# ksahlin/NGSpeciesID

Measured on AMD Instinct MI355X. Metric: reads/sec end-to-end (cluster + spoa consensus + racon x3), 750 bp ONT, higher is better.
Workload: dtype u8 / int16 / int32 DP, 64-bit bit-vectors (f64 thresholds)

## Files before the change

### ngspeciesid_amd/csrc/k_align.hip

```cpp
#include "k_align_common.h"
#include <algorithm>
#include <type_traits>

#define NEGINF (-(1 << 29))

template <int RPL>
__global__ __launch_bounds__(256) __attribute__((amdgpu_waves_per_eu(3, 4)))
void k_sg_align(AlignJob J, uint64_t* __restrict__ tb, uint64_t tb_words_per_wave, int32_t* __restrict__ bnd, uint32_t bnd_stride, uint32_t lds_per_wave, uint32_t* __restrict__ work_ctr)
{
    extern __shared__ __attribute__((aligned(16))) unsigned char smem[];
    const int lane = threadIdx.x & 63;
    const int wib = threadIdx.x >> 6;
    const uint64_t wave = (uint64_t)blockIdx.x * (blockDim.x >> 6) + wib;
    uint8_t* tgt = smem + (size_t)wib * lds_per_wave;
    const uint32_t seq_lds = (lds_per_wave - 4096) / 2;
    uint8_t* qry = tgt + seq_lds;
    uint64_t* tbblk = (uint64_t*)(tgt + 2 * (size_t)seq_lds);
    uint64_t* mytb = tb + wave * tb_words_per_wave;
    int32_t* mybnd = bnd + wave * (uint64_t)bnd_stride * 2;
    const int STRIP = 64 * RPL;

    for (;;) {
        uint32_t pq = 0; if (lane == 0) pq = atomicAdd(work_ctr, 1u);
        const uint64_t px = (uint32_t)__builtin_amdgcn_readfirstlane((int)pq);
// ... 183 lines not shown
static int32_t plan16(ngsid_ctx* ctx, uint64_t npairs, uint32_t max_qlen, uint32_t max_tlen, StripPlan* L)
{
    return plan_strips(ctx, (const void*)k_sg_align16<RP>, 2 * RP, 127, npairs, max_qlen, max_tlen, L);
}
template <int RP>
static int32_t launch16(ngsid_ctx* ctx, const AlignJob& job, const StripPlan& L, hipStream_t st, uint32_t* ctr, uint64_t* tb, int32_t* bnd)
{
    { ProfScope ps_(ctx, st == ctx->stream ? "k_sg_align" : "k_sg_align_side", st);
      hipLaunchKernelGGL((k_sg_align16<RP>), dim3((unsigned)(L.nwaves / L.wpb)), dim3(64 * L.wpb), (size_t)L.wpb * L.lds_per_wave, st,
                         job, tb, L.words, bnd, L.bnd_stride, L.lds_per_wave, ctr); }
    HIPCHK(ctx, hipGetLastError());
    return NGSID_OK;
}

struct PairedPlan { uint64_t words_half, nwaves; uint32_t seq_lds; size_t lds; };
template <int R>
static int32_t plan16p(ngsid_ctx* ctx, uint64_t npairs, uint32_t max_tlen, PairedPlan* L)
{
    L->seq_lds = (std::max<uint32_t>(max_tlen, 64u * R) + 15u) & ~15u;
    L->lds = 4 * (size_t)L->seq_lds + 4096;
    L->words_half = ((uint64_t)max_tlen + 63) * 64;
    return plan_waves(ctx, (const void*)k_sg_align16p<R>, 1, L->lds, (npairs + 1) / 2, 2 * L->words_half * 8, &L->nwaves);
}

__global__ __launch_bounds__(256)
void k_pair_bins(AlignJob J, const uint32_t* __restrict__ list, const uint32_t* __restrict__ count, int R, uint8_t* __restrict__ bin_of, uint32_t* __restrict__ bin_cnt )
{
    const uint32_t k = blockIdx.x * blockDim.x + threadIdx.x;
    const int lane = threadIdx.x & 63;
    int bin = -1;
    if (k < *count) {
        const uint64_t p = list[k]; const uint32_t qi = J.qidx[p];
        const int n = (int)(J.qoff[qi + 1] - J.qoff[qi]);
        bin = n >= 1 ? (n - 1) % R : 0;
        bin_of[k] = (uint8_t)bin;
    }
    for (int b = 0; b < PBINS; ++b) {
// ... 12 lines not shown
void k_bin_scatter(const uint32_t* __restrict__ list, const uint32_t* __restrict__ count, const uint8_t* __restrict__ bin_of, const uint32_t* __restrict__ bin_off, uint32_t* __restrict__ cursor, uint32_t* __restrict__ sorted)
{
    const uint32_t k = blockIdx.x * blockDim.x + threadIdx.x;
    const int lane = threadIdx.x & 63;
    const int bin = k < *count ? (int)bin_of[k] : -1;
    for (int b = 0; b < PBINS; ++b) {
        const unsigned long long mk = __ballot(bin == b);
        if (!mk) continue;
        const int leader = (int)__builtin_ctzll(mk);
        uint32_t base = 0; if (lane == leader) base = atomicAdd(&cursor[b], (uint32_t)__popcll(mk));
        base = __shfl(base, leader);
        if (bin == b) sorted[bin_off[b] + base + __popcll(mk & ((1ull << lane) - 1))] = list[k];
    }
}

template <int R>
static int32_t launch16p(ngsid_ctx* ctx, const AlignJob& job, int cls, uint32_t max_tlen, hipStream_t st, uint64_t* tb)
{
    const uint64_t n = job.npairs;
    const size_t ints = 4 * PBINS + 8;
    if (ctx->aln_pint.n < 4 * ints) HIPCHK(ctx, ctx->aln_pint.alloc(4 * ints));
    if (ctx->aln_psorted.n < 4 * n) HIPCHK(ctx, ctx->aln_psorted.reserve(4 * n));
    if (ctx->aln_pbin.n < 4 * n) HIPCHK(ctx, ctx->aln_pbin.reserve(4 * n));
    uint32_t* ibase = ctx->aln_pint.p + cls * ints; uint32_t* sorted = ctx->aln_psorted.p + (size_t)cls * n; uint8_t* bin_of = ctx->aln_pbin.p + (size_t)cls * n;
    const uint32_t* list = ctx->aln_cls.p + (size_t)cls * n; const uint32_t* count = ctx->aln_ctr.p + 8 + cls;
    uint32_t* bin_cnt = ibase, *bin_off = ibase + PBINS, *item_off = bin_off + PBINS + 1, *cursor = item_off + PBINS + 1, *wctr = cursor + PBINS;
    HIPCHK(ctx, hipMemsetAsync(ibase, 0, (size_t)(4 * PBINS + 8) * sizeof(uint32_t), st));
    const unsigned nb = (unsigned)((n + 255) / 256);
    hipLaunchKernelGGL(k_pair_bins, dim3(nb), dim3(256), 0, st, job, list, count, R, bin_of, bin_cnt);
    hipLaunchKernelGGL(k_bin_offsets, dim3(1), dim3(64), 0, st, (const uint32_t*)bin_cnt, bin_off, item_off, cursor);
    hipLaunchKernelGGL(k_bin_scatter, dim3(nb), dim3(256), 0, st, list, count, (const uint8_t*)bin_of, (const uint32_t*)bin_off, cursor, sorted);
    HIPCHK(ctx, hipGetLastError());
    PairedPlan L; int32_t rc = plan16p<R>(ctx, n, max_tlen, &L); if (rc) return rc;
    HIPCHK(ctx, hipFuncSetAttribute((const void*)k_sg_align16p<R>, hipFuncAttributeMaxDynamicSharedMemorySize, (int)L.lds));
    { ProfScope ps_(ctx, st == ctx->stream ? "k_sg_align" : "k_sg_align_side", st);
      hipLaunchKernelGGL((k_sg_align16p<R>), dim3((unsigned)L.nwaves), dim3(64), L.lds, st, job, (const uint32_t*)sorted, (const uint32_t*)bin_off, (const uint32_t*)item_off, tb, L.words_half, L.seq_lds, wctr); }
    HIPCHK(ctx, hipGetLastError());
    return NGSID_OK;
}


#define NCLS 5
struct AlignClass { uint32_t bound; int rp, r, side; };
constexpr AlignClass kAlignClass[NCLS] = {{256, 2, 4, 0}, {512, 4, 8, 1}, {768, 6, 12, -1}, {896, 7, 14, 2}, {0xffffffffu, 8, 0, 3}};

template <class F>
static int32_t with_class(int c, F&& f)
{
    switch (c) {
        case 0: return f(std::integral_constant<int, 0>{});
        case 1: return f(std::integral_constant<int, 1>{});
// ... 23 lines not shown
        if (cls == c) lists[(size_t)c * J.npairs + base + __popcll(m & ((1ull << lane) - 1))] = (uint32_t)p;
    }
}

int32_t ngsid_partition_pairs(ngsid_ctx* ctx, const AlignJob& job, uint32_t long_len)
{
    const uint64_t n = job.npairs;
    if (ctx->aln_ctr.n < 16) HIPCHK(ctx, ctx->aln_ctr.alloc(16));
    if (ctx->aln_cls.n < (size_t)(NCLS + 1) * n) HIPCHK(ctx, ctx->aln_cls.reserve((size_t)(NCLS + 1) * n));
    HIPCHK(ctx, hipMemsetAsync(ctx->aln_ctr.p, 0, 16 * sizeof(uint32_t), ctx->stream));
    hipLaunchKernelGGL(k_pair_classes, dim3((unsigned)((n + 255) / 256)), dim3(256), 0, ctx->stream, job, ctx->aln_cls.p, ctx->aln_ctr.p + 8, long_len);
    HIPCHK(ctx, hipGetLastError());
    return NGSID_OK;
}

static int32_t launch_classes(ngsid_ctx* ctx, const AlignJob& job, uint32_t max_qlen, uint32_t max_tlen, uint32_t min_qlen, uint32_t long_len)
{
    const uint64_t n = job.npairs;
    { int32_t rc = ngsid_partition_pairs(ctx, job, long_len); if (rc) return rc; }
    { int32_t rc = ngsid_side_streams(ctx); if (rc) return rc; }
    const bool paired = ngsid_opt(ctx, "align_paired", 1) != 0;
    bool used[NCLS]; uint64_t tbo[NCLS + 1] = {0}, bo[NCLS + 1] = {0};
    for (int c = 0; c < NCLS; ++c) {
        used[c] = (c == 0 || max_qlen > kAlignClass[c - 1].bound) && min_qlen <= std::min(max_qlen, kAlignClass[c].bound);
        uint64_t words = 0, bwords = 0;
        if (used[c]) {
            int32_t rc = with_class(c, [&](auto C) -> int32_t {
                constexpr AlignClass K = kAlignClass[decltype(C)::value];
                if constexpr (K.r > 0) {
                    if (paired) { PairedPlan P; int32_t r = plan16p<K.r>(ctx, n, max_tlen, &P); words = P.nwaves * 2 * P.words_half; return r; }
                }
                StripPlan L; int32_t r = plan16<K.rp>(ctx, n, std::min(max_qlen, K.bound), max_tlen, &L); words = L.nwaves * L.words; bwords = L.nwaves * 2ull * L.bnd_stride; return r;
            });
            if (rc) return rc;
        }
        tbo[c + 1] = tbo[c] + words; bo[c + 1] = bo[c] + bwords;
    }
    if (ctx->tb.n < tbo[NCLS]) HIPCHK(ctx, ctx->tb.reserve(tbo[NCLS]));
    if (ctx->bnd.n < bo[NCLS]) HIPCHK(ctx, ctx->bnd.reserve(bo[NCLS]));
    HIPCHK(ctx, hipEventRecord(ctx->ev_fork, ctx->stream));
    for (int i = 0; i < 4; ++i) HIPCHK(ctx, hipStreamWaitEvent(ctx->side[i], ctx->ev_fork, 0));
    for (int on_main = 0; on_main < 2; ++on_main)
        for (int c = 0; c < NCLS; ++c) {
            if (!used[c] || (kAlignClass[c].side < 0) != (on_main == 1)) continue;
            const hipStream_t st = kAlignClass[c].side < 0 ? ctx->stream : ctx->side[kAlignClass[c].side];
            int32_t rc = with_class(c, [&](auto C) -> int32_t {
                constexpr AlignClass K = kAlignClass[decltype(C)::value];
                if constexpr (K.r > 0) {
                    if (paired) return launch16p<K.r>(ctx, job, c, max_tlen, st, ctx->tb.p + tbo[c]);
                }
                AlignJob jc = job; jc.pair_list = ctx->aln_cls.p + (size_t)c * n; jc.npairs_dev = ctx->aln_ctr.p + 8 + c;
                StripPlan L; int32_t r = plan16<K.rp>(ctx, n, std::min(max_qlen, K.bound), max_tlen, &L); if (r) return r;
                return launch16<K.rp>(ctx, jc, L, st, ctx->aln_ctr.p + 1 + c, ctx->tb.p + tbo[c], ctx->bnd.p + bo[c]);
            });
            if (rc) return rc;
        }
    for (int i = 0; i < 4; ++i) { HIPCHK(ctx, hipEventRecord(ctx->ev_join[i], ctx->side[i])); HIPCHK(ctx, hipStreamWaitEvent(ctx->stream, ctx->ev_join[i], 0)); }
    return NGSID_OK;
}

bool ngsid_align16_applicable(const AlignJob& job, uint32_t max_qlen, uint32_t max_tlen, int max_open)
{
    return max_qlen <= NGSID_ALIGN16_MAXLEN && max_tlen <= NGSID_ALIGN16_MAXLEN && job.match >= 0 && job.match <= 4 && job.mismatch <= 0 && job.mismatch >= -8 &&
           job.ext >= 0 && job.ext <= 4 && max_open >= 0 && max_open <= 16;
}

__global__ __launch_bounds__(256) void k_align_cells(AlignJob J, unsigned long long* __restrict__ stat)
{
    const uint64_t np = J.npairs_dev ? (uint64_t)*J.npairs_dev : J.npairs;
    unsigned long long c = 0;
    for (uint64_t x = (uint64_t)blockIdx.x * 256 + threadIdx.x; x < np; x += (uint64_t)gridDim.x * 256) {
        const uint64_t p = J.pair_list ? J.pair_list[x] : x; const uint32_t qi = J.qidx[p], ti = J.tidx[p];
        c += (unsigned long long)(J.qoff[qi + 1] - J.qoff[qi]) * (unsigned long long)(J.toff[ti + 1] - J.toff[ti]);
    }
#pragma unroll
    for (int d = 32; d >= 1; d >>= 1) c += __shfl_xor(c, d);
    __shared__ unsigned long long part[4];
    if ((threadIdx.x & 63) == 0) part[threadIdx.x >> 6] = c;
    __syncthreads();
    if (threadIdx.x == 0) atomicAdd(stat, part[0] + part[1] + part[2] + part[3]);
}

int32_t ngsid_launch_align(ngsid_ctx* ctx, const AlignJob& job, uint32_t max_qlen, uint32_t max_tlen, int max_open, uint32_t min_qlen)
{
    if (job.npairs == 0) return NGSID_OK;
    if (ctx->prof && ctx->stat.p && !job.bp) { hipLaunchKernelGGL(k_align_cells, dim3((unsigned)std::min<uint64_t>(1024, (job.npairs + 255) / 256)), dim3(256), 0, ctx->stream, job, ctx->stat.p + 1); HIPCHK(ctx, hipGetLastError()); }
    if (job.npairs > 0xf0000000ull) NGSID_FAIL(ctx, NGSID_ERR_ARG, "more than 2^32 pairs in one aligner call");
    if (max_tlen > NGSID_MAX_READ_LEN || max_qlen > NGSID_MAX_READ_LEN) NGSID_FAIL(ctx, NGSID_ERR_TOO_LONG, "sequence longer than %d in aligner", NGSID_MAX_READ_LEN);
    if (job.k > 64) NGSID_FAIL(ctx, NGSID_ERR_ARG, "window k > 64 unsupported");
    if (!job.ops && !ngsid_opt(ctx, "align32", 0)) {
        const uint32_t q16 = std::min<uint32_t>(max_qlen, NGSID_ALIGN16_MAXLEN), t16 = std::min<uint32_t>(max_tlen, NGSID_ALIGN16_MAXLEN);
        const bool has_long = max_qlen > q16 || max_tlen > t16;
        if (ngsid_align16_applicable(job, q16, t16, max_open)) {
            if (job.npairs >= 4096 && q16 > 256 && !job.pair_list && !ngsid_opt(ctx, "align_noclass", 0)) {
                int32_t rc = launch_classes(ctx, job, q16, t16, min_qlen, has_long ? NGSID_ALIGN16_MAXLEN : 0);
                if (rc || !has_long) return rc;
                AlignJob jl = job; jl.pair_list = ctx->aln_cls.p + (size_t)NCLS * job.npairs; jl.npairs_dev = ctx->aln_ctr.p + 8 + NCLS;
                return launch_rpl<16>(ctx, jl, max_qlen, max_tlen, true);
            }
            if (!has_long) {
                int c = 0; while (max_qlen > kAlignClass[c].bound) ++c;
                return with_class(c, [&](auto C) -> int32_t {
                    constexpr int RP = kAlignClass[decltype(C)::value].rp;
                    StripPlan L; int32_t rc = plan16<RP>(ctx, job.npairs, max_qlen, max_tlen, &L); if (rc) return rc;
                    if (ctx->aln_ctr.n < 16) HIPCHK(ctx, ctx->aln_ctr.alloc(16));
                    HIPCHK(ctx, hipMemsetAsync(ctx->aln_ctr.p, 0, sizeof(uint32_t), ctx->stream));
                    if (ctx->tb.n < L.nwaves * L.words) HIPCHK(ctx, ctx->tb.alloc(L.nwaves * L.words));
                    if (ctx->bnd.n < L.nwaves * 2ull * L.bnd_stride) HIPCHK(ctx, ctx->bnd.alloc(L.nwaves * 2ull * L.bnd_stride));
                    return launch16<RP>(ctx, job, L, ctx->stream, ctx->aln_ctr.p, ctx->tb.p, ctx->bnd.p);
                });
// ... 11 lines not shown
```

### ngspeciesid_amd/csrc/k_align16p.hip

```cpp
#include "k_align_common.h"
#include <type_traits>

static_assert(-(NEG16) + 4  + 16  + 4  * 896  < 32768, "packed sign-bit flags of k_sg_align16p would wrap");
__device__ __forceinline__ int pp_bfi(int mask_s, int a, int b) { int d; asm("v_bfi_b32 %0, %1, %2, %3" : "=v"(d) : "s"(mask_s), "v"(a), "v"(b)); return d; }
__device__ __forceinline__ int pp_perm(int a, int b, int sel_s) { int d; asm("v_perm_b32 %0, %1, %2, %3" : "=v"(d) : "v"(a), "v"(b), "s"(sel_s)); return d; }
__device__ __forceinline__ int pp_sel(int mask, int a, int b) { return (a & mask) | (b & ~mask); }

template <int R>
struct Planes {
    const uint64_t* tb;
    __device__ SgCell at(int i, int j) const { const int l = i / R; return SgCell{l >> 3, j + l, l & 7, i - l * R}; }
    __device__ const uint64_t* block(int grp, int tt) const { return tb + (uint64_t)tt * 64 + grp * 8; }
    __device__ int flags(uint64_t word, int r) const {
        const unsigned x = (unsigned)(word >> (32 * (r >> 3) + (r & 7)));
        return (int)(~(x & 1u) & 1u) | (int)(~(x >> 7) & 2u) | (int)(~(x >> 14) & 4u) | (int)(~(x >> 21) & 8u);
    }
};

template <int R>
__global__ __launch_bounds__(64) __attribute__((amdgpu_waves_per_eu(2, 4)))
void k_sg_align16p(AlignJob J, const uint32_t* __restrict__ sorted, const uint32_t* __restrict__ bin_off , const uint32_t* __restrict__ item_off ,
                   uint64_t* __restrict__ tb, uint64_t tb_words_per_wave , uint32_t seq_lds, uint32_t* __restrict__ work_ctr)
{
    extern __shared__ __attribute__((aligned(16))) unsigned char smem[];
    const int lane = threadIdx.x;
    uint8_t* tgt0 = smem; uint8_t* tgt1 = tgt0 + seq_lds; uint8_t* qry0 = tgt1 + seq_lds; uint8_t* qry1 = qry0 + seq_lds;
    uint64_t* tbblk = (uint64_t*)(smem + 4 * (size_t)seq_lds);
    uint64_t* mytb0 = tb + (uint64_t)blockIdx.x * tb_words_per_wave * 2; uint64_t* mytb1 = mytb0 + tb_words_per_wave;
    constexpr int NA = 2 * ((R + 7) / 8);
    const uint32_t nitems = item_off[PBINS];

    for (;;) {
        uint32_t pq = 0; if (lane == 0) pq = atomicAdd(work_ctr, 1u);
        const uint32_t kq = (uint32_t)__builtin_amdgcn_readfirstlane((int)pq);
        if (kq >= nitems) break;
// ... 12 lines not shown
        if (deg0) sg_degenerate(J, p0, n0, m0, lane);
        if (deg1) sg_degenerate(J, p1, n1, m1, lane);
        const int own_p = ((n0 > 0 ? n0 : 1) - 1) % R;
        if (deg0) { n0 = 0; m0 = 0; }
        if (deg1) { n1 = 0; m1 = 0; }
        if (deg0 && (deg1 || !have1)) continue;
        unsigned wild = 0;
        for (int x = lane; x < m0; x += 64) { const uint8_t v = perm_letter(t0[x]); tgt0[x] = v; wild |= v; }
        for (int x = lane; x < n0; x += 64) { const uint8_t v = perm_letter(q0[x]); qry0[x] = v; wild |= v; }
        for (int x = lane; x < m1; x += 64) { const uint8_t v = perm_letter(t1[x]); tgt1[x] = v; wild |= v; }
        for (int x = lane; x < n1; x += 64) { const uint8_t v = perm_letter(q1[x]); qry1[x] = v; wild |= v; }
        const bool nowild = __ballot((wild & 0x7Cu) != 0) == 0;
        __builtin_amdgcn_fence(__ATOMIC_RELEASE, "workgroup");
        __builtin_amdgcn_wave_barrier();

        const int OPEN2 = sgpr(PK(J.open[p0], J.open[p1])), NOPEN2 = sgpr(PK(-J.open[p0], -J.open[p1])), EXT2 = sgpr(PK(J.ext, J.ext));
        const int MATCHO2 = PK(J.match + J.open[p0], J.match + J.open[p1]), NDIFF2 = sgpr(PK(J.mismatch - J.match, J.mismatch - J.match));
        const int ONE2 = sgpr(0x00010001);
        constexpr int SGN = 0x0B0A0908;
        constexpr int SEL0 = 0x06040200, SEL1 = 0x07050301;
        const int mmax = m0 > m1 ? m0 : m1;
        const int steps = mmax + 63;
        const int own_lane0 = n0 > 0 ? (n0 - 1) / R : -1, own_lane1 = n1 > 0 ? (n1 - 1) / R : -1;
        int bestRowV0 = -(1 << 29), bestRowJ0 = 0, bestRowV1 = -(1 << 29), bestRowJ1 = 0;
        int hl2[R], e2[R], qc2[R], nwq2[R];
        const int i0 = lane * R;
#pragma unroll
        for (int r = 0; r < R; ++r) {
            const int i = i0 + r;
            const int ca = i < n0 ? qry0[i] : 0x7C, cb = i < n1 ? qry1[i] : 0x7C;
            qc2[r] = PK(ca & 3, cb & 3); nwq2[r] = PK((ca & 0x7C) ? 0 : 0xffff, (cb & 0x7C) ? 0 : 0xffff);
            hl2[r] = NOPEN2; e2[r] = PK(NEG16, NEG16);
        }

        auto forward = [&](auto OPc, auto NWc) {
            constexpr int OWN_P = decltype(OPc)::value; constexpr bool NOWILD = decltype(NWc)::value;
            int hdiag2 = NOPEN2;
            int send_h = NOPEN2, send_f = PK(NEG16, NEG16);
            int keyRow0 = (int)0x80000000u, keyRow1 = (int)0x80000000u; const int jinv0 = 0xFFFF + lane;
            auto step = [&](int tau, auto STc) {
                constexpr bool STEADY = decltype(STc)::value;
                const int j = tau - lane;
                const int hup = __builtin_amdgcn_update_dpp(NOPEN2, send_h, 0x138, 0xf, 0xf, false), fup = __builtin_amdgcn_update_dpp(PK(NEG16, NEG16), send_f, 0x138, 0xf, 0xf, false);
                const bool a0 = STEADY || (j >= 0 && j < m0), a1 = STEADY || (j >= 0 && j < m1);
                const int l0 = tgt0[STEADY ? j : (a0 ? j : 0)], l1 = tgt1[STEADY ? j : (a1 ? j : 0)];
                const int tc2 = PK(l0 & 3, l1 & 3);
                int nwt2 = 0; if constexpr (!NOWILD) nwt2 = PK((a0 && !(l0 & 0x7C)) ? 0xffff : 0, (a1 && !(l1 & 0x7C)) ? 0xffff : 0);
                const int am2 = STEADY ? -1 : PK(a0 ? 0xffff : 0, a1 ? 0xffff : 0);
                int hu2 = hup, f2 = fup, hd2 = hdiag2;
                int acc[NA], cap2 = 0;
#pragma unroll
                for (int r = 0; r < R; ++r) {
                    const int e_ext = pk_sub_i16_s(e2[r], EXT2); const int E = pk_max_i16(e_ext, hl2[r]);
                    const int f_ext = pk_sub_i16_s(f2, EXT2); const int F = pk_max_i16(f_ext, hu2);
                    const int z = pk_min_u16_s(qc2[r] ^ tc2, ONE2);
                    int sc = pk_mad_i16_sv(z, NDIFF2, MATCHO2);
                    if constexpr (!NOWILD) { const int nw = nwq2[r] & nwt2; sc = pp_sel(nw, sc, OPEN2); }
                    const int d = pk_add_i16(hd2, sc);
                    const int mx = pk_max_i16(E, F); const int h = pk_max_i16(d, mx);
                    const int g = pk_sub_i16_s(h, OPEN2);
                    const int s0 = pk_sub_i16(d, h), s1 = pk_sub_i16(E, mx), s2 = pk_sub_i16(e_ext, E), s3 = pk_sub_i16(f_ext, F);
                    const int pa = pp_perm(s1, s0, SGN), pb = pp_perm(s3, s2, SGN);
                    int& a01 = acc[2 * (r >> 3)]; int& a23 = acc[2 * (r >> 3) + 1];
                    if ((r & 7) == 0) { a01 = pa & 0x01010101; a23 = pb & 0x01010101; }
                    else { a01 = pp_bfi(0x01010101 << (r & 7), pa, a01); a23 = pp_bfi(0x01010101 << (r & 7), pb, a23); }
                    hd2 = hl2[r];
                    hl2[r] = STEADY ? g : pp_sel(am2, g, hl2[r]);
                    e2[r] = E;
                    hu2 = g; f2 = F;
                    if (r == OWN_P) cap2 = g;
                }
                unsigned long long w0 = 0, w1 = 0;
#pragma unroll
                for (int k = 0; k < NA / 2; ++k) {
                    w0 |= (unsigned long long)(unsigned)pp_perm(acc[2 * k + 1], acc[2 * k], SEL0) << (32 * k);
                    w1 |= (unsigned long long)(unsigned)pp_perm(acc[2 * k + 1], acc[2 * k], SEL1) << (32 * k);
                }
                mytb0[(uint64_t)tau * 64 + lane] = w0;
                mytb1[(uint64_t)tau * 64 + lane] = w1;
                if (STEADY) { hdiag2 = hup; send_h = hu2; send_f = f2; }
                else { hdiag2 = pp_sel(am2, hup, hdiag2); send_h = pp_sel(am2, hu2, send_h); send_f = pp_sel(am2, f2, send_f); }
                if (STEADY) {
                    const int jinv = jinv0 - tau;
                    keyRow0 = max(keyRow0, (int)(((unsigned)cap2 << 16) | (unsigned)jinv));
                    keyRow1 = max(keyRow1, (int)(((unsigned)cap2 & 0xFFFF0000u) | (unsigned)jinv));
                } else {
                    const int v0 = LO16(cap2), v1 = HI16(cap2);
                    const bool b0_ = a0 && lane == own_lane0 && v0 > bestRowV0; bestRowV0 = b0_ ? v0 : bestRowV0; bestRowJ0 = b0_ ? j : bestRowJ0;
                    const bool b1_ = a1 && lane == own_lane1 && v1 > bestRowV1; bestRowV1 = b1_ ? v1 : bestRowV1; bestRowJ1 = b1_ ? j : bestRowJ1;
                }
            };
            const int mmin = m0 < m1 ? m0 : m1;
            const int st_lo = 63 < steps ? 63 : steps, st_hi = mmin > st_lo ? (mmin < steps ? mmin : steps) : st_lo;
            int tau = 0;
            for (; tau < st_lo; ++tau) step(tau, std::false_type{});
            for (; tau + 1 < st_hi; tau += 2) { step(tau, std::true_type{}); step(tau + 1, std::true_type{}); }
            for (; tau < st_hi; ++tau) step(tau, std::true_type{});
            if (st_hi > st_lo) {
                const int v0 = keyRow0 >> 16, v1 = keyRow1 >> 16;
                if (lane == own_lane0 && v0 > bestRowV0) { bestRowV0 = v0; bestRowJ0 = 0xFFFF - (keyRow0 & 0xFFFF); }
                if (lane == own_lane1 && v1 > bestRowV1) { bestRowV1 = v1; bestRowJ1 = 0xFFFF - (keyRow1 & 0xFFFF); }
            }
            for (; tau < steps; ++tau) step(tau, std::false_type{});
        };
        switch (own_p) {
#define PCASE(k) case k: if (nowild) forward(std::integral_constant<int, (R > k ? k : 0)>{}, std::true_type{}); else forward(std::integral_constant<int, (R > k ? k : 0)>{}, std::false_type{}); break;
            PCASE(0) PCASE(1) PCASE(2) PCASE(3) PCASE(4) PCASE(5) PCASE(6) PCASE(7) PCASE(8) PCASE(9) PCASE(10) PCASE(11) PCASE(12) PCASE(13) PCASE(14)
#undef PCASE
            default: if (nowild) forward(std::integral_constant<int, (R > 15 ? 15 : 0)>{}, std::true_type{}); else forward(std::integral_constant<int, (R > 15 ? 15 : 0)>{}, std::false_type{}); break;
        }
        bestRowV0 += LO16(OPEN2); bestRowV1 += HI16(OPEN2);
        int bestColV0 = -(1 << 29), bestColI0 = 0x7fffffff, bestColV1 = -(1 << 29), bestColI1 = 0x7fffffff;
#pragma unroll
        for (int r = 0; r < R; ++r) {
            const int i = i0 + r; const int v0 = LO16(hl2[r]) + LO16(OPEN2), v1 = HI16(hl2[r]) + HI16(OPEN2);
            if (i < n0 && v0 > bestColV0) { bestColV0 = v0; bestColI0 = i; }
            if (i < n1 && v1 > bestColV1) { bestColV1 = v1; bestColI1 = i; }
        }
        __builtin_amdgcn_fence(__ATOMIC_RELEASE, "workgroup");
        __builtin_amdgcn_s_waitcnt(0);
        __builtin_amdgcn_fence(__ATOMIC_ACQUIRE, "workgroup");

        const AlignJob* Jt = sg_cold_job();
        for (int half = 0; half < 2; ++half) {
            const uint64_t p = half ? p1 : p0; const int n = half ? n1 : n0, m = half ? m1 : m0;
            if (n <= 0) continue;
            int rowV = half ? bestRowV1 : bestRowV0, rowJ = half ? bestRowJ1 : bestRowJ0;
#pragma unroll
            for (int d = 32; d >= 1; d >>= 1) { int ov = __shfl_xor(rowV, d), oj = __shfl_xor(rowJ, d); if (ov > rowV) { rowV = ov; rowJ = oj; } }
            int colV = half ? bestColV1 : bestColV0, colI = half ? bestColI1 : bestColI0;
#pragma unroll
            for (int d = 32; d >= 1; d >>= 1) { int ov = __shfl_xor(colV, d), oi = __shfl_xor(colI, d); if (ov > colV || (ov == colV && oi < colI)) { colV = ov; colI = oi; } }
            int ei = n - 1, ej = rowJ, best = rowV;
            if (colV > best) { best = colV; ei = colI; ej = m - 1; }
            ei = sgpr(ei); ej = sgpr(ej); best = sgpr(best);
            sg_walk(Jt, Planes<R>{half ? mytb1 : mytb0}, tbblk, half ? qry1 : qry0, half ? tgt1 : tgt0, p, n, m, ei, ej, best, lane);
            __builtin_amdgcn_wave_barrier();
        }
    }
}

template __global__ void k_sg_align16p<4>(AlignJob, const uint32_t*, const uint32_t*, const uint32_t*, uint64_t*, uint64_t, uint32_t, uint32_t*);
template __global__ void k_sg_align16p<8>(AlignJob, const uint32_t*, const uint32_t*, const uint32_t*, uint64_t*, uint64_t, uint32_t, uint32_t*);
template __global__ void k_sg_align16p<12>(AlignJob, const uint32_t*, const uint32_t*, const uint32_t*, uint64_t*, uint64_t, uint32_t, uint32_t*);
template __global__ void k_sg_align16p<14>(AlignJob, const uint32_t*, const uint32_t*, const uint32_t*, uint64_t*, uint64_t, uint32_t, uint32_t*);
```

### ngspeciesid_amd/csrc/k_align_common.h

```cpp
#pragma once
#include "ngsid_internal.h"

template <int RP> __global__ void k_sg_align16(AlignJob J, uint64_t* tb, uint64_t tb_words_per_wave, int32_t* bnd, uint32_t bnd_stride, uint32_t lds_per_wave, uint32_t* work_ctr);
#define PBINS 32
template <int R> __global__ void k_sg_align16p(AlignJob J, const uint32_t* sorted, const uint32_t* bin_off, const uint32_t* item_off, uint64_t* tb, uint64_t tb_words_per_wave, uint32_t seq_lds, uint32_t* work_ctr);

#define NEG16 (-20000)
#define PKOP2(name, mnem) __device__ __forceinline__ int name(int a, int b) { int d; asm(mnem " %0, %1, %2" : "=v"(d) : "v"(a), "v"(b)); return d; }
PKOP2(pk_sub_i16, "v_pk_sub_i16")
PKOP2(pk_add_i16, "v_pk_add_i16")
PKOP2(pk_max_i16, "v_pk_max_i16")
PKOP2(pk_sub_u16, "v_pk_sub_u16")
#define PKOP2S(name, mnem) __device__ __forceinline__ int name(int a, int b) { int d; asm(mnem " %0, %1, %2" : "=v"(d) : "v"(a), "s"(b)); return d; }
PKOP2S(pk_sub_i16_s, "v_pk_sub_i16")
PKOP2S(pk_min_u16_s, "v_pk_min_u16")
__device__ __forceinline__ int pk_mad_i16_sv(int a, int b_s, int c) { int d; asm("v_pk_mad_i16 %0, %1, %2, %3" : "=v"(d) : "v"(a), "s"(b_s), "v"(c)); return d; }
__device__ __forceinline__ int sgpr(int x) { return __builtin_amdgcn_readfirstlane(x); }
__device__ __forceinline__ uint8_t perm_letter(uint8_t c) {
    const int b = ngsid_bcode(c);
    if (b < 4) return (uint8_t)(b | ((c & 0x20) ? 0x80 : 0));
    if ((c & 0x7C) == 0) { const int x = c & 3; const int up = x == 0 ? 'A' : x == 1 ? 'C' : x == 2 ? 'G' : 'T'; return (uint8_t)((c & 0x80) ? (up | 0x20) : up); }
    return c;
}
__device__ __forceinline__ int PK(int lo, int hi) { return (lo & 0xffff) | (hi << 16); }
// ... 142 lines not shown
```

### ngspeciesid_amd/csrc/ngsid_api.hip

```cpp
#include "ngsid_internal.h"
#include "../../include/ngsid_merge_schedule.h"
#include "../../include/ngsid_tables.h"
#include <math.h>
#include <algorithm>

extern "C" uint32_t ngsid_abi_version(void) { return 2u; }

static char g_static_err[256] = "";
extern "C" const char* ngsid_last_error(ngsid_ctx* ctx) { return ctx ? ctx->err : g_static_err; }

namespace {
struct DevPool { std::mutex mu; std::multimap<unsigned long long, void*> free_; size_t cached = 0; int contexts = 0; size_t live = 0, peak = 0;
                 struct Upload { size_t bs; void* q; size_t bq; void* off; size_t bo; }; std::map<void*, Upload> uploads;
};
DevPool g_pool;
const size_t POOL_LIMIT = (size_t)48 << 30;
const size_t POOL_HEADROOM = (size_t)3 << 30;
struct PoolBlocks { void* p[3] = {nullptr, nullptr, nullptr}; size_t b[3] = {0, 0, 0}; bool owned = true; ~PoolBlocks() { if (owned) for (int i = 0; i < 3; ++i) if (p[i]) ngsid_pool_free(p[i], b[i]); } };
inline size_t pool_class(size_t b) { if (b < 4096) return 4096; int sh = 63 - __builtin_clzll((unsigned long long)b) - 3; size_t m = ((size_t)1 << sh) - 1; return (b + m) & ~m; }
inline unsigned long long pool_key(int dev, size_t cls) { return ((unsigned long long)dev << 56) | (unsigned long long)cls; }
}
thread_local ngsid_ctx* g_ngsid_tls_ctx = nullptr;
hipError_t ngsid_pool_alloc(void** p, size_t bytes, size_t* got)
{
// ... 536 lines not shown
extern "C" int32_t ngsid_reads_release(ngsid_ctx* ctx, ngsid_reads_t* dev)
{
    if (!ctx) return NGSID_ERR_ARG;
    ApiClock api_clock_(ctx, "reads_release");
    if (!dev || dev->mem != NGSID_MEM_DEVICE) NGSID_FAIL(ctx, NGSID_ERR_ARG, "reads_release: not a device read set");
    DevPool::Upload u;
    { std::lock_guard<std::mutex> lk(g_pool.mu); auto it = g_pool.uploads.find((void*)dev->seq); if (it == g_pool.uploads.end()) NGSID_FAIL(ctx, NGSID_ERR_ARG, "reads_release: this read set was not made by ngsid_reads_upload (or was released already)"); u = it->second; g_pool.uploads.erase(it); }
    ngsid_pool_free((void*)dev->seq, u.bs); if (u.q) ngsid_pool_free(u.q, u.bq); ngsid_pool_free(u.off, u.bo);
    dev->seq = nullptr; dev->qual = nullptr; dev->off = nullptr; dev->n = 0;
    return NGSID_OK;
}

extern "C" int32_t ngsid_ctx_option(ngsid_ctx* ctx, const char* name, int64_t value)
{
    if (!ctx || !name) return NGSID_ERR_ARG;
    static const char* known[] = {"minimizers_chunk_bases", "poa_level_budget_mb", "cluster_block", "cluster_block_cap", "cluster_trunc", "cluster_seg_order", "ed_band", "ed_win_all", "align32", "align_noclass", "poa_tiles_per_cu", "minimizers_lean", "minimizers_mode", "poa_host_levels", "align_paired", "poa_out_slots", "ed_lds_pad_kb", "ed_win6", "support_budget_mb", "demux_chunk_reads", "classify_chunk_queries"};
    for (const char* k : known) if (!strcmp(k, name)) { ctx->options[name] = (long long)value; return NGSID_OK; }
    if (!strcmp(name, "touch")) {
        if (ctx->mzc_fp.n < 2) HIPCHK(ctx, ctx->mzc_fp.alloc(2));
        HIPCHK(ctx, hipMemsetAsync(ctx->mzc_fp.p + 1, 0, sizeof(unsigned long long), ctx->stream)); HIPCHK(ctx, hipStreamSynchronize(ctx->stream));
        return NGSID_OK;
    }
    if (!strcmp(name, "release_scratch")) {
        (void)hipStreamSynchronize(ctx->stream);
        ctx->tb.release(); ctx->bnd.release(); ctx->tb_long.release(); ctx->bnd_long.release(); ctx->aln_cls.release(); ctx->aln_psorted.release(); ctx->aln_pbin.release(); ctx->ed_tb.release(); ctx->ed_h.release(); ctx->ed_fail.release(); ctx->ed_fail2.release();
        ctx->poa_h.release(); ctx->poa_d.release(); ctx->poa_g.release(); ctx->poa_cov.release();
        for (auto& L : ctx->poa_lv) { L.out.release(); L.seqs.release(); L.job_final.release(); L.out_len.release(); L.out_span.release(); L.job_bb.release(); L.out_cw.release(); L.out_n.release(); L.out_cov.release(); L.job_off.release(); L.seq_idx.release(); L.flags.release(); L.job_list.release(); L.job_unit.release(); L.job_pos.release(); }
        ctx->mzc.valid = false; ctx->mzc_cnt.release(); ctx->mzc_hlen.release(); ctx->mz_off.release(); ctx->mz_scode.release(); ctx->mz_spos.release();
        ctx->pol_mzcode.release(); ctx->pol_mzpos.release(); ctx->pol_oseq.release(); ctx->pol_oqual.release(); ctx->pol_valid.release(); ctx->pol_bp.release(); ctx->pol_lay.release(); ctx->cl_cnt.release(); ctx->cls_cnt.release();
        ngsid_pool_release_all();
        return NGSID_OK;
// ... 56 lines not shown
```

### ngspeciesid_amd/csrc/ngsid_internal.h

```cpp
#pragma once
#include <hip/hip_runtime.h>
#include <stdint.h>
#include <stdio.h>
#include <string.h>
#include <stdlib.h>
#include <string>
#include <vector>
#include <map>
#include <new>
#include <mutex>
#include <chrono>
#include <memory>
#include <time.h>
#include "../../include/ngsid.h"

hipError_t ngsid_pool_alloc(void** p, size_t bytes, size_t* got);
void ngsid_pool_free(void* p, size_t bytes);
struct ngsid_ctx;
extern thread_local ngsid_ctx* g_ngsid_tls_ctx;
void ngsid_pool_release_all();
int ngsid_pool_contexts();
size_t ngsid_pool_cached_bytes();
void ngsid_pool_stats(size_t* live, size_t* peak, bool reset_peak);

// ... 126 lines not shown
                             uint32_t* h_cnt, uint32_t* h_hlen, long long* bad_read);

struct AlignJob {
    const uint8_t* qseq; const uint64_t* qoff; const uint8_t* tseq; const uint64_t* toff;
    const uint32_t* qidx; const uint32_t* tidx; uint64_t npairs;
    int match, mismatch, ext, k; const int32_t* open; const int32_t* match_id;
    int32_t* score; int32_t* ncols; int32_t* nmatch; int32_t* region;
    int32_t* bp; int bp_windows; int window; int32_t* span;
    const uint32_t* pair_list; const uint32_t* npairs_dev;
    uint8_t* ops; const uint64_t* ops_off;
    const uint32_t* pair_list2; const uint32_t* npairs_dev2;
    int clip;
};
int32_t ngsid_launch_align(ngsid_ctx* ctx, const AlignJob& job, uint32_t max_qlen, uint32_t max_tlen, int max_open = 1 << 20, uint32_t min_qlen = 0);
bool ngsid_align16_applicable(const AlignJob& job, uint32_t max_qlen, uint32_t max_tlen, int max_open);
#define NGSID_ALIGN16_MAXLEN 4000u
int32_t ngsid_partition_pairs(ngsid_ctx* ctx, const AlignJob& job, uint32_t long_len = 0);
int32_t ngsid_side_streams(ngsid_ctx* ctx);
int32_t ngsid_launch_ed_align(ngsid_ctx* ctx, const AlignJob& job, uint32_t max_qlen, uint32_t max_tlen, int32_t* dist_out);
int32_t ngsid_launch_ed_align_rec(ngsid_ctx* ctx, const AlignJob& job, uint32_t max_qlen, uint32_t max_tlen, uint32_t* rec, uint32_t stride);
enum { NGSID_REC_EQ = 1, NGSID_REC_SUB = 2 , NGSID_REC_OTHER = 6 , NGSID_REC_DEL = 7, NGSID_REC_INS = 8 };
struct OrientBufs { DevBuf<uint32_t> d_rgroup; DevBuf<double> herr, rawerr; DevBuf<uint8_t> d_orient; };
int32_t ngsid_polish_orient(ngsid_ctx* ctx, const DevReads& RD, const std::vector<std::string>& B, const std::vector<uint32_t>& h_rgroup, int k, int w, OrientBufs& S, PinVec<uint8_t>& h_orient);

typedef unsigned int ngsid_v4u __attribute__((ext_vector_type(4)));
__device__ __forceinline__ ngsid_v4u ngsid_load16_l2(const void* p) { return __builtin_nontemporal_load((const ngsid_v4u*)p); }

__device__ __forceinline__ int ngsid_bcode(uint8_t c) {
    switch (c) { case 'A': case 'a': return 0; case 'C': case 'c': return 1; case 'G': case 'g': return 2; case 'T': case 't': return 3; default: return 4; }
}
// ... 7 lines not shown
```

Before: 1.465 million.

## Add skewed-frame variant of paired int16 aligner with byte-permute score table

Adds a SKEW template variant of the paired 16-bit semi-global aligner. Each cell is rebased by i+j times the gap-extension cost, so the E/F extension subtracts disappear. When there are no wildcards, the match/mismatch score comes from a v_perm byte lookup table instead of xor/min/mad. It also raises the waves-per-EU hint for the skew variant. The variant is enabled by default only when a new overflow bound shows the skewed int16 range cannot wrap, and it adds extra per-step offset corrections and register pressure.

```diff
diff --git a/ngspeciesid_amd/csrc/k_align.hip b/ngspeciesid_amd/csrc/k_align.hip
--- a/ngspeciesid_amd/csrc/k_align.hip
+++ b/ngspeciesid_amd/csrc/k_align.hip
@@ -221,13 +221,13 @@
 }
 
 struct PairedPlan { uint64_t words_half, nwaves; uint32_t seq_lds; size_t lds; };
-template <int R>
+template <int R, bool SKEW>
 static int32_t plan16p(ngsid_ctx* ctx, uint64_t npairs, uint32_t max_tlen, PairedPlan* L)
 {
     L->seq_lds = (std::max<uint32_t>(max_tlen, 64u * R) + 15u) & ~15u;
     L->lds = 4 * (size_t)L->seq_lds + 4096;
     L->words_half = ((uint64_t)max_tlen + 63) * 64;
-    return plan_waves(ctx, (const void*)k_sg_align16p<R>, 1, L->lds, (npairs + 1) / 2, 2 * L->words_half * 8, &L->nwaves);
+    return plan_waves(ctx, (const void*)k_sg_align16p<R, SKEW>, 1, L->lds, (npairs + 1) / 2, 2 * L->words_half * 8, &L->nwaves);
 }
 
 __global__ __launch_bounds__(256)
@@ -270,7 +270,7 @@
     }
 }
 
-template <int R>
+template <int R, bool SKEW>
 static int32_t launch16p(ngsid_ctx* ctx, const AlignJob& job, int cls, uint32_t max_tlen, hipStream_t st, uint64_t* tb)
 {
     const uint64_t n = job.npairs;
@@ -287,10 +287,10 @@
     hipLaunchKernelGGL(k_bin_offsets, dim3(1), dim3(64), 0, st, (const uint32_t*)bin_cnt, bin_off, item_off, cursor);
     hipLaunchKernelGGL(k_bin_scatter, dim3(nb), dim3(256), 0, st, list, count, (const uint8_t*)bin_of, (const uint32_t*)bin_off, cursor, sorted);
     HIPCHK(ctx, hipGetLastError());
-    PairedPlan L; int32_t rc = plan16p<R>(ctx, n, max_tlen, &L); if (rc) return rc;
-    HIPCHK(ctx, hipFuncSetAttribute((const void*)k_sg_align16p<R>, hipFuncAttributeMaxDynamicSharedMemorySize, (int)L.lds));
+    PairedPlan L; int32_t rc = plan16p<R, SKEW>(ctx, n, max_tlen, &L); if (rc) return rc;
+    HIPCHK(ctx, hipFuncSetAttribute((const void*)k_sg_align16p<R, SKEW>, hipFuncAttributeMaxDynamicSharedMemorySize, (int)L.lds));
     { ProfScope ps_(ctx, st == ctx->stream ? "k_sg_align" : "k_sg_align_side", st);
-      hipLaunchKernelGGL((k_sg_align16p<R>), dim3((unsigned)L.nwaves), dim3(64), L.lds, st, job, (const uint32_t*)sorted, (const uint32_t*)bin_off, (const uint32_t*)item_off, tb, L.words_half, L.seq_lds, wctr); }
+      hipLaunchKernelGGL((k_sg_align16p<R, SKEW>), dim3((unsigned)L.nwaves), dim3(64), L.lds, st, job, (const uint32_t*)sorted, (const uint32_t*)bin_off, (const uint32_t*)item_off, tb, L.words_half, L.seq_lds, wctr); }
     HIPCHK(ctx, hipGetLastError());
     return NGSID_OK;
 }
@@ -344,12 +344,13 @@
     return NGSID_OK;
 }
 
-static int32_t launch_classes(ngsid_ctx* ctx, const AlignJob& job, uint32_t max_qlen, uint32_t max_tlen, uint32_t min_qlen, uint32_t long_len)
+static int32_t launch_classes(ngsid_ctx* ctx, const AlignJob& job, uint32_t max_qlen, uint32_t max_tlen, int max_open, uint32_t min_qlen, uint32_t long_len)
 {
     const uint64_t n = job.npairs;
     { int32_t rc = ngsid_partition_pairs(ctx, job, long_len); if (rc) return rc; }
     { int32_t rc = ngsid_side_streams(ctx); if (rc) return rc; }
     const bool paired = ngsid_opt(ctx, "align_paired", 1) != 0;
+    const bool skew = ngsid_opt(ctx, "align_skew", 1) != 0 && ngsid_align16p_skew_exact(job, max_qlen, max_tlen, max_open);
     bool used[NCLS]; uint64_t tbo[NCLS + 1] = {0}, bo[NCLS + 1] = {0};
     for (int c = 0; c < NCLS; ++c) {
         used[c] = (c == 0 || max_qlen > kAlignClass[c - 1].bound) && min_qlen <= std::min(max_qlen, kAlignClass[c].bound);
@@ -358,7 +359,7 @@
             int32_t rc = with_class(c, [&](auto C) -> int32_t {
                 constexpr AlignClass K = kAlignClass[decltype(C)::value];
                 if constexpr (K.r > 0) {
-                    if (paired) { PairedPlan P; int32_t r = plan16p<K.r>(ctx, n, max_tlen, &P); words = P.nwaves * 2 * P.words_half; return r; }
+                    if (paired) { PairedPlan P; int32_t r = skew ? plan16p<K.r, true>(ctx, n, max_tlen, &P) : plan16p<K.r, false>(ctx, n, max_tlen, &P); words = P.nwaves * 2 * P.words_half; return r; }
                 }
                 StripPlan L; int32_t r = plan16<K.rp>(ctx, n, std::min(max_qlen, K.bound), max_tlen, &L); words = L.nwaves * L.words; bwords = L.nwaves * 2ull * L.bnd_stride; return r;
             });
@@ -377,7 +378,7 @@
             int32_t rc = with_class(c, [&](auto C) -> int32_t {
                 constexpr AlignClass K = kAlignClass[decltype(C)::value];
                 if constexpr (K.r > 0) {
-                    if (paired) return launch16p<K.r>(ctx, job, c, max_tlen, st, ctx->tb.p + tbo[c]);
+                    if (paired) return skew ? launch16p<K.r, true>(ctx, job, c, max_tlen, st, ctx->tb.p + tbo[c]) : launch16p<K.r, false>(ctx, job, c, max_tlen, st, ctx->tb.p + tbo[c]);
                 }
                 AlignJob jc = job; jc.pair_list = ctx->aln_cls.p + (size_t)c * n; jc.npairs_dev = ctx->aln_ctr.p + 8 + c;
                 StripPlan L; int32_t r = plan16<K.rp>(ctx, n, std::min(max_qlen, K.bound), max_tlen, &L); if (r) return r;
@@ -393,6 +394,14 @@
 {
     return max_qlen <= NGSID_ALIGN16_MAXLEN && max_tlen <= NGSID_ALIGN16_MAXLEN && job.match >= 0 && job.match <= 4 && job.mismatch <= 0 && job.mismatch >= -8 &&
            job.ext >= 0 && job.ext <= 4 && max_open >= 0 && max_open <= 16;
+}
+
+bool ngsid_align16p_skew_exact(const AlignJob& job, uint32_t max_qlen, uint32_t max_tlen, int max_open)
+{
+    uint32_t qmax = 0;
+    for (int c = 0; c < NCLS; ++c) if (kAlignClass[c].r > 0) qmax = std::max(qmax, kAlignClass[c].bound);
+    return ngsid_align16_applicable(job, max_qlen, max_tlen, max_open) &&
+           sg16p_flag_span(job.match, job.ext, max_open, std::min(max_qlen, qmax), max_tlen, true) < 32768;
 }
 
 __global__ __launch_bounds__(256) void k_align_cells(AlignJob J, unsigned long long* __restrict__ stat)
@@ -423,7 +432,7 @@
         const bool has_long = max_qlen > q16 || max_tlen > t16;
         if (ngsid_align16_applicable(job, q16, t16, max_open)) {
             if (job.npairs >= 4096 && q16 > 256 && !job.pair_list && !ngsid_opt(ctx, "align_noclass", 0)) {
-                int32_t rc = launch_classes(ctx, job, q16, t16, min_qlen, has_long ? NGSID_ALIGN16_MAXLEN : 0);
+                int32_t rc = launch_classes(ctx, job, q16, t16, max_open, min_qlen, has_long ? NGSID_ALIGN16_MAXLEN : 0);
                 if (rc || !has_long) return rc;
                 AlignJob jl = job; jl.pair_list = ctx->aln_cls.p + (size_t)NCLS * job.npairs; jl.npairs_dev = ctx->aln_ctr.p + 8 + NCLS;
                 return launch_rpl<16>(ctx, jl, max_qlen, max_tlen, true);
diff --git a/ngspeciesid_amd/csrc/k_align16p.hip b/ngspeciesid_amd/csrc/k_align16p.hip
--- a/ngspeciesid_amd/csrc/k_align16p.hip
+++ b/ngspeciesid_amd/csrc/k_align16p.hip
@@ -1,9 +1,12 @@
 #include "k_align_common.h"
 #include <type_traits>
 
-static_assert(-(NEG16) + 4  + 16  + 4  * 896  < 32768, "packed sign-bit flags of k_sg_align16p would wrap");
+static_assert(sg16p_flag_span(4 , 4 , 16 , 896 , NGSID_ALIGN16_MAXLEN, false) < 32768, "packed sign-bit flags of k_sg_align16p would wrap");
+static_assert(sg16p_flag_span(4, 1, 16, 896, NGSID_ALIGN16_MAXLEN, true) < 32768, "the skewed frame of k_sg_align16p must hold every paired length with ext = 1");
 __device__ __forceinline__ int pp_bfi(int mask_s, int a, int b) { int d; asm("v_bfi_b32 %0, %1, %2, %3" : "=v"(d) : "s"(mask_s), "v"(a), "v"(b)); return d; }
 __device__ __forceinline__ int pp_perm(int a, int b, int sel_s) { int d; asm("v_perm_b32 %0, %1, %2, %3" : "=v"(d) : "v"(a), "v"(b), "s"(sel_s)); return d; }
+__device__ __forceinline__ int pp_permv(int a, int b, int sel_v) { int d; asm("v_perm_b32 %0, %1, %2, %3" : "=v"(d) : "v"(a), "v"(b), "v"(sel_v)); return d; }
+__device__ __forceinline__ int pk_ashr15_i16(int a) { int d; asm("v_pk_ashrrev_i16 %0, %1, %2" : "=v"(d) : "s"(0x000F000F), "v"(a)); return d; }
 __device__ __forceinline__ int pp_sel(int mask, int a, int b) { return (a & mask) | (b & ~mask); }
 
 template <int R>
@@ -17,8 +20,8 @@
     }
 };
 
-template <int R>
-__global__ __launch_bounds__(64) __attribute__((amdgpu_waves_per_eu(2, 4)))
+template <int R, bool SKEW>
+__global__ __launch_bounds__(64) __attribute__((amdgpu_waves_per_eu(SKEW ? (R <= 8 ? 4 : 3) : 2, 4)))
 void k_sg_align16p(AlignJob J, const uint32_t* __restrict__ sorted, const uint32_t* __restrict__ bin_off , const uint32_t* __restrict__ item_off ,
                    uint64_t* __restrict__ tb, uint64_t tb_words_per_wave , uint32_t seq_lds, uint32_t* __restrict__ work_ctr)
 {
@@ -61,9 +64,15 @@
         __builtin_amdgcn_fence(__ATOMIC_RELEASE, "workgroup");
         __builtin_amdgcn_wave_barrier();
 
-        const int OPEN2 = sgpr(PK(J.open[p0], J.open[p1])), NOPEN2 = sgpr(PK(-J.open[p0], -J.open[p1])), EXT2 = sgpr(PK(J.ext, J.ext));
-        const int MATCHO2 = PK(J.match + J.open[p0], J.match + J.open[p1]), NDIFF2 = sgpr(PK(J.mismatch - J.match, J.mismatch - J.match));
+        int ext = J.ext; if constexpr (SKEW) asm volatile("" : "+s"(ext));
+        const int open0 = sgpr(J.open[p0]), open1 = sgpr(J.open[p1]), skx = SKEW ? ext : 0;
+        const int NOPEN2 = sgpr(PK(-open0, -open1)), EXT2 = sgpr(PK(ext, ext));
+        const int dk0 = open0 + skx, dk1 = open1 + skx;
+        const int DIAG2 = sgpr(PK(dk0, dk1)), GSUB2 = sgpr(PK(open0 - skx, open1 - skx));
+        const int MATCHO2 = PK(J.match + dk0, J.match + dk1), NDIFF2 = sgpr(PK(J.mismatch - J.match, J.mismatch - J.match));
         const int ONE2 = sgpr(0x00010001);
+        const bool tbl_ok = SKEW && J.mismatch + dk0 >= 0 && J.mismatch + dk1 >= 0 && J.match + dk0 <= 255 && J.match + dk1 <= 255;
+        const int XX0 = sgpr((J.mismatch + dk0) * 0x01010101), XX1 = sgpr((J.mismatch + dk1) * 0x01010101), MX0 = sgpr((J.match + dk0) ^ (J.mismatch + dk0)), MX1 = sgpr((J.match + dk1) ^ (J.mismatch + dk1));
         constexpr int SGN = 0x0B0A0908;
         constexpr int SEL0 = 0x06040200, SEL1 = 0x07050301;
         const int mmax = m0 > m1 ? m0 : m1;
@@ -71,41 +80,53 @@
         const int own_lane0 = n0 > 0 ? (n0 - 1) / R : -1, own_lane1 = n1 > 0 ? (n1 - 1) / R : -1;
         int bestRowV0 = -(1 << 29), bestRowJ0 = 0, bestRowV1 = -(1 << 29), bestRowJ1 = 0;
         int hl2[R], e2[R], qc2[R], nwq2[R];
-        const int i0 = lane * R;
+        int i0 = lane * R; if constexpr (SKEW) asm volatile("" : "+v"(i0));
 #pragma unroll
         for (int r = 0; r < R; ++r) {
             const int i = i0 + r;
             const int ca = i < n0 ? qry0[i] : 0x7C, cb = i < n1 ? qry1[i] : 0x7C;
-            qc2[r] = PK(ca & 3, cb & 3); nwq2[r] = PK((ca & 0x7C) ? 0 : 0xffff, (cb & 0x7C) ? 0 : 0xffff);
-            hl2[r] = NOPEN2; e2[r] = PK(NEG16, NEG16);
+            if constexpr (SKEW) { qc2[r] = PK((ca & 3) | ((ca & 0x7C) ? 0x8000 : 0), (cb & 3) | ((cb & 0x7C) ? 0x8000 : 0)); nwq2[r] = 0; }
+            else { qc2[r] = PK(ca & 3, cb & 3); nwq2[r] = PK((ca & 0x7C) ? 0 : 0xffff, (cb & 0x7C) ? 0 : 0xffff); }
+            hl2[r] = SKEW ? PK(i * ext - open0, i * ext - open1) : NOPEN2; e2[r] = PK(NEG16, NEG16);
         }
 
         auto forward = [&](auto OPc, auto NWc) {
             constexpr int OWN_P = decltype(OPc)::value; constexpr bool NOWILD = decltype(NWc)::value;
-            int hdiag2 = NOPEN2;
+            constexpr bool TABLE = SKEW && NOWILD;
+            int hdiag2 = SKEW ? PK((i0 - 1) * ext - open0, (i0 - 1) * ext - open1) : NOPEN2;
+            if constexpr (TABLE) {
+#pragma unroll
+                for (int r = 0; r < R; ++r) qc2[r] += 0x0C040C00;
+            }
             int send_h = NOPEN2, send_f = PK(NEG16, NEG16);
             int keyRow0 = (int)0x80000000u, keyRow1 = (int)0x80000000u; const int jinv0 = 0xFFFF + lane;
             auto step = [&](int tau, auto STc) {
                 constexpr bool STEADY = decltype(STc)::value;
                 const int j = tau - lane;
-                const int hup = __builtin_amdgcn_update_dpp(NOPEN2, send_h, 0x138, 0xf, 0xf, false), fup = __builtin_amdgcn_update_dpp(PK(NEG16, NEG16), send_f, 0x138, 0xf, 0xf, false);
+                const int top2 = SKEW ? PK(tau * ext - open0, tau * ext - open1) : NOPEN2;
+                const int hup = __builtin_amdgcn_update_dpp(top2, send_h, 0x138, 0xf, 0xf, false), fup = __builtin_amdgcn_update_dpp(PK(NEG16, NEG16), send_f, 0x138, 0xf, 0xf, false);
                 const bool a0 = STEADY || (j >= 0 && j < m0), a1 = STEADY || (j >= 0 && j < m1);
                 const int l0 = tgt0[STEADY ? j : (a0 ? j : 0)], l1 = tgt1[STEADY ? j : (a1 ? j : 0)];
-                const int tc2 = PK(l0 & 3, l1 & 3);
+                const int tc2 = TABLE ? 0 : PK(l0 & 3, l1 & 3);
+                int tb0 = 0, tb1 = 0; if constexpr (TABLE) { tb0 = XX0 ^ (MX0 << ((l0 << 3) & 31)); tb1 = XX1 ^ (MX1 << ((l1 << 3) & 31)); }
                 int nwt2 = 0; if constexpr (!NOWILD) nwt2 = PK((a0 && !(l0 & 0x7C)) ? 0xffff : 0, (a1 && !(l1 & 0x7C)) ? 0xffff : 0);
                 const int am2 = STEADY ? -1 : PK(a0 ? 0xffff : 0, a1 ? 0xffff : 0);
                 int hu2 = hup, f2 = fup, hd2 = hdiag2;
                 int acc[NA], cap2 = 0;
 #pragma unroll
                 for (int r = 0; r < R; ++r) {
-                    const int e_ext = pk_sub_i16_s(e2[r], EXT2); const int E = pk_max_i16(e_ext, hl2[r]);
-                    const int f_ext = pk_sub_i16_s(f2, EXT2); const int F = pk_max_i16(f_ext, hu2);
-                    const int z = pk_min_u16_s(qc2[r] ^ tc2, ONE2);
-                    int sc = pk_mad_i16_sv(z, NDIFF2, MATCHO2);
-                    if constexpr (!NOWILD) { const int nw = nwq2[r] & nwt2; sc = pp_sel(nw, sc, OPEN2); }
+                    const int e_ext = SKEW ? e2[r] : pk_sub_i16_s(e2[r], EXT2); const int E = pk_max_i16(e_ext, hl2[r]);
+                    const int f_ext = SKEW ? f2 : pk_sub_i16_s(f2, EXT2); const int F = pk_max_i16(f_ext, hu2);
+                    int sc;
+                    if constexpr (TABLE) sc = pp_permv(tb1, tb0, qc2[r]);
+                    else {
+                        const int z = pk_min_u16_s(qc2[r] ^ tc2, ONE2);
+                        sc = pk_mad_i16_sv(z, NDIFF2, MATCHO2);
+                    }
+                    if constexpr (!NOWILD) { const int nw = SKEW ? (~pk_ashr15_i16(qc2[r]) & nwt2) : (nwq2[r] & nwt2); sc = pp_sel(nw, sc, DIAG2); }
                     const int d = pk_add_i16(hd2, sc);
                     const int mx = pk_max_i16(E, F); const int h = pk_max_i16(d, mx);
-                    const int g = pk_sub_i16_s(h, OPEN2);
+                    const int g = pk_sub_i16_s(h, GSUB2);
                     const int s0 = pk_sub_i16(d, h), s1 = pk_sub_i16(E, mx), s2 = pk_sub_i16(e_ext, E), s3 = pk_sub_i16(f_ext, F);
                     const int pa = pp_perm(s1, s0, SGN), pb = pp_perm(s3, s2, SGN);
                     int& a01 = acc[2 * (r >> 3)]; int& a23 = acc[2 * (r >> 3) + 1];
@@ -113,7 +134,7 @@
                     else { a01 = pp_bfi(0x01010101 << (r & 7), pa, a01); a23 = pp_bfi(0x01010101 << (r & 7), pb, a23); }
                     hd2 = hl2[r];
                     hl2[r] = STEADY ? g : pp_sel(am2, g, hl2[r]);
-                    e2[r] = E;
+                    e2[r] = (SKEW && !STEADY) ? pp_sel(am2, E, e2[r]) : E;
                     hu2 = g; f2 = F;
                     if (r == OWN_P) cap2 = g;
                 }
@@ -127,6 +148,7 @@
                 mytb1[(uint64_t)tau * 64 + lane] = w1;
                 if (STEADY) { hdiag2 = hup; send_h = hu2; send_f = f2; }
                 else { hdiag2 = pp_sel(am2, hup, hdiag2); send_h = pp_sel(am2, hu2, send_h); send_f = pp_sel(am2, f2, send_f); }
+                if constexpr (SKEW) cap2 = pk_sub_i16_s(cap2, sgpr(PK(tau * ext, tau * ext)));
                 if (STEADY) {
                     const int jinv = jinv0 - tau;
                     keyRow0 = max(keyRow0, (int)(((unsigned)cap2 << 16) | (unsigned)jinv));
@@ -151,16 +173,17 @@
             for (; tau < steps; ++tau) step(tau, std::false_type{});
         };
         switch (own_p) {
-#define PCASE(k) case k: if (nowild) forward(std::integral_constant<int, (R > k ? k : 0)>{}, std::true_type{}); else forward(std::integral_constant<int, (R > k ? k : 0)>{}, std::false_type{}); break;
+#define PCASE(k) case k: if (SKEW ? (nowild && tbl_ok) : nowild) forward(std::integral_constant<int, (R > k ? k : 0)>{}, std::true_type{}); else forward(std::integral_constant<int, (R > k ? k : 0)>{}, std::false_type{}); break;
             PCASE(0) PCASE(1) PCASE(2) PCASE(3) PCASE(4) PCASE(5) PCASE(6) PCASE(7) PCASE(8) PCASE(9) PCASE(10) PCASE(11) PCASE(12) PCASE(13) PCASE(14)
 #undef PCASE
-            default: if (nowild) forward(std::integral_constant<int, (R > 15 ? 15 : 0)>{}, std::true_type{}); else forward(std::integral_constant<int, (R > 15 ? 15 : 0)>{}, std::false_type{}); break;
-        }
-        bestRowV0 += LO16(OPEN2); bestRowV1 += HI16(OPEN2);
+            default: if (SKEW ? (nowild && tbl_ok) : nowild) forward(std::integral_constant<int, (R > 15 ? 15 : 0)>{}, std::true_type{}); else forward(std::integral_constant<int, (R > 15 ? 15 : 0)>{}, std::false_type{}); break;
+        }
+        bestRowV0 += open0 - skx * (n0 - own_lane0); bestRowV1 += open1 - skx * (n1 - own_lane1);
         int bestColV0 = -(1 << 29), bestColI0 = 0x7fffffff, bestColV1 = -(1 << 29), bestColI1 = 0x7fffffff;
+        if constexpr (SKEW) { i0 = lane * R; asm volatile("" : "+v"(i0)); }
 #pragma unroll
         for (int r = 0; r < R; ++r) {
-            const int i = i0 + r; const int v0 = LO16(hl2[r]) + LO16(OPEN2), v1 = HI16(hl2[r]) + HI16(OPEN2);
+            const int i = i0 + r; const int v0 = LO16(hl2[r]) + open0 - skx * (i + m0), v1 = HI16(hl2[r]) + open1 - skx * (i + m1);
             if (i < n0 && v0 > bestColV0) { bestColV0 = v0; bestColI0 = i; }
             if (i < n1 && v1 > bestColV1) { bestColV1 = v1; bestColI1 = i; }
         }
@@ -187,7 +210,11 @@
     }
 }
 
-template __global__ void k_sg_align16p<4>(AlignJob, const uint32_t*, const uint32_t*, const uint32_t*, uint64_t*, uint64_t, uint32_t, uint32_t*);
-template __global__ void k_sg_align16p<8>(AlignJob, const uint32_t*, const uint32_t*, const uint32_t*, uint64_t*, uint64_t, uint32_t, uint32_t*);
-template __global__ void k_sg_align16p<12>(AlignJob, const uint32_t*, const uint32_t*, const uint32_t*, uint64_t*, uint64_t, uint32_t, uint32_t*);
-template __global__ void k_sg_align16p<14>(AlignJob, const uint32_t*, const uint32_t*, const uint32_t*, uint64_t*, uint64_t, uint32_t, uint32_t*);
+template __global__ void k_sg_align16p<4, false>(AlignJob, const uint32_t*, const uint32_t*, const uint32_t*, uint64_t*, uint64_t, uint32_t, uint32_t*);
+template __global__ void k_sg_align16p<4, true>(AlignJob, const uint32_t*, const uint32_t*, const uint32_t*, uint64_t*, uint64_t, uint32_t, uint32_t*);
+template __global__ void k_sg_align16p<8, false>(AlignJob, const uint32_t*, const uint32_t*, const uint32_t*, uint64_t*, uint64_t, uint32_t, uint32_t*);
+template __global__ void k_sg_align16p<8, true>(AlignJob, const uint32_t*, const uint32_t*, const uint32_t*, uint64_t*, uint64_t, uint32_t, uint32_t*);
+template __global__ void k_sg_align16p<12, false>(AlignJob, const uint32_t*, const uint32_t*, const uint32_t*, uint64_t*, uint64_t, uint32_t, uint32_t*);
+template __global__ void k_sg_align16p<12, true>(AlignJob, const uint32_t*, const uint32_t*, const uint32_t*, uint64_t*, uint64_t, uint32_t, uint32_t*);
+template __global__ void k_sg_align16p<14, false>(AlignJob, const uint32_t*, const uint32_t*, const uint32_t*, uint64_t*, uint64_t, uint32_t, uint32_t*);
+template __global__ void k_sg_align16p<14, true>(AlignJob, const uint32_t*, const uint32_t*, const uint32_t*, uint64_t*, uint64_t, uint32_t, uint32_t*);
diff --git a/ngspeciesid_amd/csrc/k_align_common.h b/ngspeciesid_amd/csrc/k_align_common.h
--- a/ngspeciesid_amd/csrc/k_align_common.h
+++ b/ngspeciesid_amd/csrc/k_align_common.h
@@ -3,9 +3,13 @@
 
 template <int RP> __global__ void k_sg_align16(AlignJob J, uint64_t* tb, uint64_t tb_words_per_wave, int32_t* bnd, uint32_t bnd_stride, uint32_t lds_per_wave, uint32_t* work_ctr);
 #define PBINS 32
-template <int R> __global__ void k_sg_align16p(AlignJob J, const uint32_t* sorted, const uint32_t* bin_off, const uint32_t* item_off, uint64_t* tb, uint64_t tb_words_per_wave, uint32_t seq_lds, uint32_t* work_ctr);
+template <int R, bool SKEW> __global__ void k_sg_align16p(AlignJob J, const uint32_t* sorted, const uint32_t* bin_off, const uint32_t* item_off, uint64_t* tb, uint64_t tb_words_per_wave, uint32_t seq_lds, uint32_t* work_ctr);
 
 #define NEG16 (-20000)
+constexpr long long sg16p_flag_span(int match, int ext, int open, long long qlen, long long tlen, bool skew)
+{
+    return -(long long)(NEG16) + ext + open + match * (qlen < tlen ? qlen : tlen) + (skew ? (qlen + tlen + 1) * ext : 0);
+}
 #define PKOP2(name, mnem) __device__ __forceinline__ int name(int a, int b) { int d; asm(mnem " %0, %1, %2" : "=v"(d) : "v"(a), "v"(b)); return d; }
 PKOP2(pk_sub_i16, "v_pk_sub_i16")
 PKOP2(pk_add_i16, "v_pk_add_i16")
diff --git a/ngspeciesid_amd/csrc/ngsid_api.hip b/ngspeciesid_amd/csrc/ngsid_api.hip
--- a/ngspeciesid_amd/csrc/ngsid_api.hip
+++ b/ngspeciesid_amd/csrc/ngsid_api.hip
@@ -574,7 +574,7 @@
 extern "C" int32_t ngsid_ctx_option(ngsid_ctx* ctx, const char* name, int64_t value)
 {
     if (!ctx || !name) return NGSID_ERR_ARG;
-    static const char* known[] = {"minimizers_chunk_bases", "poa_level_budget_mb", "cluster_block", "cluster_block_cap", "cluster_trunc", "cluster_seg_order", "ed_band", "ed_win_all", "align32", "align_noclass", "poa_tiles_per_cu", "minimizers_lean", "minimizers_mode", "poa_host_levels", "align_paired", "poa_out_slots", "ed_lds_pad_kb", "ed_win6", "support_budget_mb", "demux_chunk_reads", "classify_chunk_queries"};
+    static const char* known[] = {"minimizers_chunk_bases", "poa_level_budget_mb", "cluster_block", "cluster_block_cap", "cluster_trunc", "cluster_seg_order", "ed_band", "ed_win_all", "align32", "align_noclass", "poa_tiles_per_cu", "minimizers_lean", "minimizers_mode", "poa_host_levels", "align_paired", "align_skew", "poa_out_slots", "ed_lds_pad_kb", "ed_win6", "support_budget_mb", "demux_chunk_reads", "classify_chunk_queries"};
     for (const char* k : known) if (!strcmp(k, name)) { ctx->options[name] = (long long)value; return NGSID_OK; }
     if (!strcmp(name, "touch")) {
         if (ctx->mzc_fp.n < 2) HIPCHK(ctx, ctx->mzc_fp.alloc(2));
diff --git a/ngspeciesid_amd/csrc/ngsid_internal.h b/ngspeciesid_amd/csrc/ngsid_internal.h
--- a/ngspeciesid_amd/csrc/ngsid_internal.h
+++ b/ngspeciesid_amd/csrc/ngsid_internal.h
@@ -164,6 +164,7 @@
 };
 int32_t ngsid_launch_align(ngsid_ctx* ctx, const AlignJob& job, uint32_t max_qlen, uint32_t max_tlen, int max_open = 1 << 20, uint32_t min_qlen = 0);
 bool ngsid_align16_applicable(const AlignJob& job, uint32_t max_qlen, uint32_t max_tlen, int max_open);
+bool ngsid_align16p_skew_exact(const AlignJob& job, uint32_t max_qlen, uint32_t max_tlen, int max_open);
 #define NGSID_ALIGN16_MAXLEN 4000u
 int32_t ngsid_partition_pairs(ngsid_ctx* ctx, const AlignJob& job, uint32_t long_len = 0);
 int32_t ngsid_side_streams(ngsid_ctx* ctx);
```

After: 1.508 million (median of 6 runs). 1.03x the previous value.
